# linghaosong/Sextans

Measured on AMD Instinct MI355X. Metric: SpMM GFLOP/s + achieved HBM GB/s (fp32, N=16) at 1/2/4/8 MI355X, higher is better.
Workload: dtype f32; 1 GPU; config4: synthetic CSR 4000000x4000000, Poisson(40) nnz/row, U(-1,1) fp32, N=16, alpha=0.85, beta=-2.06, column-major B/C, seed 4; M=4000000, K=4000000, N=16, nnz=159999547, parallelism=1 GPU

## Files before the change

### sextans_amd/csrc/engine_launch.h

```cpp
#pragma once
#include "engine_state.h"

namespace sxe {

constexpr int kBlock = 256;
constexpr int kWideMaxDict = 576;

void preload_device_code();

void launch_repack(int width, const float *dB, int64_t ldb, float *dBp, int K, int col_base, int ntiles, hipStream_t s, int k_begin = 0,
                   int k_end = -1, int ncols = -1, const unsigned char *touched = nullptr);
void launch_repack_perm(sextans_engine *h, const float *dB, int64_t ldb, float *dBp, int col_base, int ntiles, int ncols, hipStream_t s);
void launch_tiles_to_colmajor(const float *tiles, float *C, int64_t ldc, int M, int col0, int ntiles, int ncols, hipStream_t s);

inline Operands on_panels(const sextans_engine *h, Operands o) {
    o.B = h->d_Bp; o.ldb = h->K; o.layout = BLayout::kPanels;
    return o;
}

void launch_rowgroup(sextans_engine *h, int width, const Operands &o, int ntiles, int row_end, const unsigned char *skip,
                     const int *groups = nullptr, int ngroups = 0);
int launch_panel(sextans_engine *h, int width, const Operands &o, int ntiles, int blk_begin, int blk_end);
enum class V2Order {
    kNatural,
    kBricks,
    kReordered,
    kPositions
};
struct PanelV2 {
    int H = 1;
    V2Order order = V2Order::kNatural;
    int blk_begin = 0, blk_end = -1;
    int last_cols = 16;
    bool dict_blocks_only = false;
};
int launch_panel_v2(sextans_engine *h, const Operands &o, int nsuper, const PanelV2 &a = {});
void launch_window(sextans_engine *h, const Operands &o, int ntiles, int wave_begin, int wave_end);
void launch_colwise(sextans_engine *h, const Operands &o, int N, int row_end);
void launch_chains(sextans_engine *h, const std::vector<Seg> &plan, const Operands &o, int c0, int c1, bool permuted_panels = false);
void launch_hub_pieces(sextans_engine *h, int width, const sextans_engine::PieceTable &t, const Operands &o, int ntiles, int col0, int v0,
                       int v1, const int *colpos = nullptr);
void launch_fold(sextans_engine *h, const sextans_engine::PieceTable &t, int hub0, int hub1, int N, const Operands &o);
void launch_transpose(bool aligned, bool to_cm, const float *src, float *dst, int64_t ld_rm, int64_t ld_cm, int rows, int cols, hipStream_t s);

void launch_rowgroup_bf16(sextans_engine *h, int width, const OperandsBf16 &o, int ntiles);
void launch_hub_pieces_bf16(sextans_engine *h, int width, const sextans_engine::PieceTable &t, const OperandsBf16 &o, int ntiles, int col0, int v0, int v1);
void launch_fold_bf16(sextans_engine *h, const sextans_engine::PieceTable &t, int N, const OperandsBf16 &o);
void launch_widen(const uint16_t *src, int64_t lds, float *dst, int64_t ldd, int64_t rows, int cols, hipStream_t s);
void launch_round(const float *src, int64_t lds, uint16_t *dst, int64_t ldd, int64_t rows, int cols, hipStream_t s);

void launch_chan_unpack_b(const float *ch, int64_t chan_len, int64_t colsize, int num_ch_b, int K, int N, float *B, hipStream_t s);
void launch_chan_unpack_c(const float *ch, int64_t chan_len, int64_t colsize, int M, int N, float *C, hipStream_t s);
void launch_chan_pack_c(const float *C, int M, int N, int64_t chan_len, int64_t colsize, float pad, float *ch, hipStream_t s);

void launch_slab_rows(bool scatter, float *tiles, int64_t tile_stride, const int *rows, int sub, int n, float *slab, int64_t slab_stride, int ntiles, hipStream_t s);

std::vector<Seg> widest_first(int N, int widest);
inline std::vector<Seg> wide_first(int N) { return widest_first(N, 32); }
inline std::vector<Seg> bf16_tiles(int N) { return widest_first(N, 64); }
enum class MainKernel { kRowgroup, kPanel, kWindow, kPanelV2 };
const char *kernel_name(MainKernel main, bool hubs, bool dense);
const char *with_rowblocks(sextans_engine *h, const char *name);

}
```

### sextans_amd/csrc/engine_launch.hip

```cpp
#include <algorithm>

#include "chan_kernels.h"
#include "dispatch.h"
#include "engine_launch.h"
#include "reorder_kernels.h"
#include "spmm_bf16_kernels.h"
#include "spmm_colwise_kernel.h"
#include "spmm_csr_kernels.h"
#include "spmm_panel_v2.h"
#include "spmm_window_kernel.h"

static_assert(sxe::kBlock == sx::kBlock && sxe::kWideMaxDict == sx::kWideMaxDict, "engine_launch.h repeats two constants of the kernel headers");

namespace {
__global__ __launch_bounds__(256) void transpose_tiles(const float *__restrict__ src, int64_t ld_src, float *__restrict__ dst, int64_t ld_dst, int rows, int cols) {
    __shared__ float t[32][33];
    const int c0 = blockIdx.x * 32, r0 = blockIdx.y * 32, tx = threadIdx.x & 31, ty = threadIdx.x >> 5;
    for (int i = ty; i < 32; i += 8)
        if (r0 + i < rows && c0 + tx < cols) t[i][tx] = src[(int64_t)(r0 + i) * ld_src + c0 + tx];
    __syncthreads();
    for (int i = ty; i < 32; i += 8)
        if (c0 + i < cols && r0 + tx < rows) dst[(int64_t)(c0 + i) * ld_dst + r0 + tx] = t[tx][i];
}
template <bool TO_CM, int CW>
// ... 30 lines not shown
        });
    }
}
}

namespace sxe {

void preload_device_code() {
    hipFuncAttributes fa;
    (void)hipFuncGetAttributes(&fa, reinterpret_cast<const void *>(&sx::repack_b_panels<16>));
    (void)hipGetLastError();
}

void launch_repack(int width, const float *dB, int64_t ldb, float *dBp, int K, int col_base, int ntiles, hipStream_t s, int k_begin,
                   int k_end, int ncols, const unsigned char *touched) {
    if (k_end < 0) k_end = K;
    if (k_end <= k_begin) return;
    if (ncols < 0) ncols = ntiles * width;
    dim3 grid((unsigned)((k_end - k_begin + sx::kBlock - 1) / sx::kBlock), (unsigned)ntiles);
    by_width(width, [&](auto L) {
        hipLaunchKernelGGL(sx::repack_b_panels<4 * decltype(L)::value>, grid, dim3(sx::kBlock), 0, s, dB, ldb, dBp, K, col_base, k_begin, k_end, ncols, touched);
    });
}

void launch_repack_perm(sextans_engine *h, const float *dB, int64_t ldb, float *dBp, int col_base, int ntiles, int ncols, hipStream_t s) {
    hipLaunchKernelGGL(sx::repack_b_panels_perm, dim3((unsigned)((h->col_hi - h->col_lo + sx::kBlock - 1) / sx::kBlock), (unsigned)ntiles), dim3(sx::kBlock), 0, s,
                       dB, ldb, dBp, h->K, col_base, h->cluster.d_colpos, h->col_lo, h->col_hi, ncols, h->mat.d_touched);
}

void launch_tiles_to_colmajor(const float *tiles, float *C, int64_t ldc, int M, int col0, int ntiles, int ncols, hipStream_t s) {
    hipLaunchKernelGGL(sx::tiles_to_colmajor, dim3((unsigned)((M + sx::kBlock - 1) / sx::kBlock), (unsigned)ntiles), dim3(sx::kBlock), 0, s, tiles, C, ldc, M, col0, ncols);
}

static int64_t b_stride(const sextans_engine *h, const Operands &o, int NT) { return o.layout == BLayout::kPanels ? (int64_t)h->K * NT : o.ldb; }

void launch_rowgroup(sextans_engine *h, int width, const Operands &o, int ntiles, int row_end, const unsigned char *skip, const int *groups, int ngroups) {
    by_width(width, [&](auto L) {
        constexpr int LPR = decltype(L)::value, RB = sx::kBlock / LPR, CH = 2048;
        const int nrowblk = groups ? ngroups * std::max(1, 128 / RB) : (row_end - o.row_base + RB - 1) / RB;
        if (nrowblk <= 0) return;
        const unsigned nwg = (unsigned)nrowblk * (unsigned)ntiles;
        with_bool(h->opt_exact, [&](auto EX) { with_bool(h->opt_stage, [&](auto ST) { with_bool(o.layout == BLayout::kRowMajor, [&](auto RM) {
            hipLaunchKernelGGL((sx::spmm_csr_rowgroup<LPR, CH, decltype(EX)::value, decltype(ST)::value, decltype(RM)::value>), dim3(nwg), dim3(sx::kBlock), 0,
                               o.s, h->m_rp, h->m_rp + 1, h->m_ci, h->m_v, o.B, b_stride(h, o, 4 * LPR), o.C_in, o.ldc_in, o.C_out, o.ldc, o.row_base, row_end, ntiles, nrowblk,
                               o.alpha, o.beta, (int)h->opt_xcd, skip, groups);
        }); }); });
    });
}

int launch_panel(sextans_engine *h, int width, const Operands &o, int ntiles, int blk_begin, int blk_end) {
    const int nblk = blk_end - blk_begin;
    if (nblk <= 0) return SEXTANS_OK;
    if (int rc = restore_plan_streams(h)) return rc;
    by_width(width, [&](auto L) {
        constexpr int LPR = decltype(L)::value, RB = sx::kBlock / LPR, NT = 4 * LPR;
        const unsigned nwg = (unsigned)nblk * (unsigned)ntiles;
        const int xcd = (int)h->opt_xcd;
        const int pad_rows = h->ps.d_ioff ? sx::kWidePadRows : 1;
        const int panel_floats = (h->ps.plan_pad_row + pad_rows) * NT;
        const int tile_floats = NT * (RB + 1);
        const size_t lds = (size_t)(panel_floats > tile_floats ? panel_floats : tile_floats) * sizeof(int);
        auto go = [&](auto kern) {
            hipLaunchKernelGGL(kern, dim3(nwg), dim3(sx::kBlock), lds, o.s, (const int2 *)h->ps.d_row_off.get(), h->ps.d_lidx,
                               h->ps.d_pcol32, h->ps.d_pval, h->ps.d_blk_row, h->ps.d_dict_ptr, h->ps.d_dict, h->ps.plan_dict_stride, o.B,
                               b_stride(h, o, NT), o.C_in, o.ldc_in, o.C_out, o.ldc, ntiles, nblk, o.alpha, o.beta, xcd, panel_floats,
                               (long long *)h->d_dbg.get(), blk_begin, o.row_base, (const unsigned char *)h->split.d_skip.get(), (const int2 *)h->ps.d_ioff.get(), pad_rows);
        };
        with_bool(h->opt_exact, [&](auto EX) {
            constexpr bool E = decltype(EX)::value;
            if (h->ps.plan_mixed) go(sx::spmm_csr_panel<LPR, E, true>);
            else if (o.layout == BLayout::kColMajor) go(sx::spmm_csr_panel<LPR, E, false, true>);
            else go(sx::spmm_csr_panel<LPR, E, false>);
        });
    });
    return SEXTANS_OK;
}

namespace {
constexpr bool kReorderedContiguous = true;

struct V2Variant {
    int H, NB; bool BCOL, TIMED = false; int DCAP = 9; bool CROW = false, BIG = false; int SETS = 1, RM = 0;
    bool operator==(const V2Variant &o) const {
        return H == o.H && NB == o.NB && BCOL == o.BCOL && TIMED == o.TIMED && DCAP == o.DCAP && CROW == o.CROW && BIG == o.BIG && SETS == o.SETS && RM == o.RM;
    }
};
struct V2Launch {
    int nb, tpw, ngrp, xcd;
    size_t lds;
    int64_t pstride;
    const int *dict, *slot_row;
    const unsigned char *skip;
    V2Variant v;
};

const sextans_engine::PanelState &v2_plan(const sextans_engine *h, V2Order order) { return order == V2Order::kNatural ? h->ps : h->cluster.psc; }

V2Launch plan_panel_v2(const sextans_engine *h, const Operands &o, int nsuper, int nblk, const PanelV2 &a) {
    V2Launch d{};
    const int H = a.H;
    const bool bcol = o.layout == BLayout::kColMajor, rm = o.layout == BLayout::kRowMajor;
    const sextans_engine::PanelState &P = v2_plan(h, a.order);
    d.slot_row = (a.order == V2Order::kBricks || a.order == V2Order::kReordered) ? h->cluster.d_slot_row : nullptr;
    d.skip = a.order == V2Order::kPositions ? nullptr : (const unsigned char *)h->split.d_skip.get();
    const bool crow = a.order == V2Order::kReordered || a.order == V2Order::kPositions;
    const int64_t mean_len = h->M > 0 ? h->m_nnz / h->M : 0;
    int nb = mean_len + 8 <= 32 ? 2 : mean_len + 8 <= 64 ? 4 : 6;
    {
        const int nb_max = std::max(1, (P.plan_max_row + 15) / 16);
        if (nb_max <= nb) nb = nb_max <= 2 ? 2 : nb_max <= 3 ? 3 : nb_max <= 4 ? 4 : 6;
        else if (nb == 2 && nb_max == 3) nb = 3;
    }
    d.nb = nb;
    const bool big = H == 1 && bcol && nb > 2;
    int tpw = (int)h->opt_tiles_per_wg;
    if (tpw <= 0 && big) {
        tpw = std::min<int>(nsuper, std::max<int>(1, (int)(((int64_t)nblk * nsuper + 2 * h->num_cus - 1) / ((int64_t)2 * h->num_cus))));
    } else if (tpw <= 0 && rm && P.plan_sets == 2 && nsuper >= 4) {
        tpw = 1;
    } else if (tpw <= 0) {
        const int64_t rounds = (int64_t)nblk * nsuper / ((int64_t)8 * h->num_cus);
        tpw = (int)std::max<int64_t>(1, std::min<int64_t>(nsuper, rounds));
    }
    d.tpw = std::min(tpw, nsuper);
    d.ngrp = (nsuper + d.tpw - 1) / d.tpw;
    d.pstride = b_stride(h, o, 16);
    d.dict = (rm && crow && h->cluster.d_dict_nat) ? h->cluster.d_dict_nat : P.d_dict;
    const bool small_panel = H == 1 && !bcol && P.plan_pad_row == 5 * 64;
    d.lds = small_panel ? (size_t)(5 * 64 + sx::kWidePadRows) * 64 : (size_t)H * sx::kWideHalfBytes;
    d.xcd = crow && h->opt_reordered_xcd >= 0 ? (int)h->opt_reordered_xcd : (crow && nsuper <= 2 && !kReorderedContiguous) ? 0 : (int)h->opt_xcd;
    V2Variant &v = d.v;
    if (H > 1) { v = {H, 6, bcol}; return d; }
    v = {1, nb, bcol};
    const bool small_dict = bcol && P.plan_max_dict <= 5 * 64 && h->opt_small_v2 != 0;
    if (h->opt_phase_timing && h->d_dbg && h->opt_exact && P.plan_sets == 1) {
        v.TIMED = true;
        if (small_dict && nb == 3) { v.DCAP = 5; return d; }
        if (bcol) { v.NB = 2; return d; }
        if (nb == 6 && !crow && !small_panel) return d;
        if (nb == 2 && !crow && small_panel) { v.DCAP = 5; return d; }
        v.TIMED = false;
    }
    if (small_dict) { v.NB = nb == 3 ? 3 : 2; v.DCAP = 5; }
    else if (big) { v.NB = nb <= 4 ? 4 : 6; v.BIG = true; }
    else if (bcol) v.NB = 2;
    else {
        if (rm) { v.CROW = true; v.RM = (int64_t)h->M * std::max(o.ldc, o.ldc_in) * 4 >= ((int64_t)1 << 32) ? 2 : 1; }
        else v.CROW = crow;
        if (P.plan_sets == 2) { v.NB = 2; v.SETS = 2; }
        else if (small_panel) { v.NB = nb >= 3 ? 3 : 2; v.DCAP = 5; }
    }
    return d;
}

template <int H, int NB, bool BCOL, bool TIMED = false, int DCAP = 9, bool CROW = false, bool BIG = false, int SETS = 1, int RM = 0>
struct V2K {
    static constexpr V2Variant v{H, NB, BCOL, TIMED, DCAP, CROW, BIG, SETS, RM};
    template <class Go>
    static int launch(bool exact, Go &go) {
        if constexpr (TIMED) return go(sx::spmm_csr_panel_v2<H, NB, true, BCOL, TIMED, DCAP, CROW, BIG, SETS, RM>);
        else return with_bool(exact, [&](auto EX) { return go(sx::spmm_csr_panel_v2<H, NB, decltype(EX)::value, BCOL, TIMED, DCAP, CROW, BIG, SETS, RM>); });
    }
};
template <class... Ks>
struct V2List {
    template <class Go>
    static int launch(const V2Variant &v, bool exact, Go &go) {
        int rc = SEXTANS_ERR_STATE;
        const bool found = ((Ks::v == v ? (rc = Ks::launch(exact, go), true) : false) || ...);
        if (!found) g_last_error = "spmm_csr_panel_v2: no instantiation for the variant decided";
        return rc;
    }
};
template <int NB, int DCAP, int SETS, int RM>
using V2Rm = V2K<1, NB, false, false, DCAP, true, false, SETS, RM>;
using PanelV2Kernels = V2List<
    V2K<2, 6, true>, V2K<2, 6, false>,
    V2K<1, 3, true, true, 5>, V2K<1, 2, true, true>, V2K<1, 6, false, true>, V2K<1, 2, false, true, 5>,
    V2K<1, 3, true, false, 5>, V2K<1, 2, true, false, 5>,
    V2K<1, 4, true, false, 9, false, true>, V2K<1, 6, true, false, 9, false, true>,
    V2K<1, 2, true>,
    V2Rm<2, 9, 2, 1>, V2Rm<3, 5, 1, 1>, V2Rm<2, 5, 1, 1>, V2Rm<2, 9, 1, 1>, V2Rm<3, 9, 1, 1>, V2Rm<4, 9, 1, 1>, V2Rm<6, 9, 1, 1>,
    V2Rm<2, 9, 2, 2>, V2Rm<3, 5, 1, 2>, V2Rm<2, 5, 1, 2>, V2Rm<2, 9, 1, 2>, V2Rm<3, 9, 1, 2>, V2Rm<4, 9, 1, 2>, V2Rm<6, 9, 1, 2>,
    V2K<1, 2, false, false, 9, true, false, 2>, V2K<1, 2, false, false, 9, false, false, 2>,
    V2K<1, 3, false, false, 5, true>, V2K<1, 2, false, false, 5, true>,
    V2K<1, 3, false, false, 5>, V2K<1, 2, false, false, 5>,
    V2K<1, 2, false, false, 9, true>, V2K<1, 3, false, false, 9, true>, V2K<1, 4, false, false, 9, true>, V2K<1, 6, false, false, 9, true>,
    V2K<1, 2, false>, V2K<1, 3, false>, V2K<1, 4, false>, V2K<1, 6, false>>;
}

int launch_panel_v2(sextans_engine *h, const Operands &o, int nsuper, const PanelV2 &a) {
    const sextans_engine::PanelState &P = v2_plan(h, a.order);
    const int blk_end = a.blk_end < 0 ? P.plan_nblk : a.blk_end;
    const int nblk = a.dict_blocks_only ? P.n_dict_blocks : blk_end - a.blk_begin;
    if (nblk <= 0 || nsuper <= 0) return SEXTANS_OK;
    if (a.order == V2Order::kNatural)
        if (int rc = restore_plan_streams(h)) return rc;
    const V2Launch d = plan_panel_v2(h, o, nsuper, nblk, a);
    auto go = [&](auto kern) -> int {
        if (int rc = allow_big_lds(h, reinterpret_cast<const void *>(kern), (int)d.lds)) return rc;
        hipLaunchKernelGGL(kern, dim3((unsigned)nblk * (unsigned)d.ngrp), dim3(sx::kBlock), d.lds, o.s, (const int2 *)P.d_row_off.get(),
                           P.d_lidx, P.d_pval, P.d_blk_row, P.d_dict_ptr, d.dict, P.plan_dict_stride, o.B, d.pstride, o.C_in, o.ldc_in, o.C_out, o.ldc, nsuper, d.tpw, nblk, o.alpha, o.beta, d.xcd,
                           P.plan_pad_row, a.blk_begin, o.row_base, d.skip, (long long *)h->d_dbg.get(), d.slot_row, (const int2 *)P.d_ioff.get(), a.last_cols, a.dict_blocks_only ? (const int *)P.d_dict_blocks.get() : (const int *)nullptr);
        return SEXTANS_OK;
    };
    return PanelV2Kernels::launch(d.v, h->opt_exact != 0, go);
}

namespace {
template <bool SCATTER>
__global__ __launch_bounds__(256) void slab_rows(float *tiles, int64_t tile_stride, const int *__restrict__ rows, int sub, int n, float *slab, int64_t slab_stride) {
    const int64_t idx = (int64_t)blockIdx.x * 256 + threadIdx.x;
    const int i = (int)(idx >> 2), q = (int)(idx & 3), t = blockIdx.y;
    if (i >= n) return;
    sx::f32x4 *a = reinterpret_cast<sx::f32x4 *>(tiles + (int64_t)t * tile_stride + (int64_t)(rows[i] - sub) * 16 + 4 * q);
    sx::f32x4 *b = reinterpret_cast<sx::f32x4 *>(slab + (int64_t)t * slab_stride + (int64_t)i * 16 + 4 * q);
    if (SCATTER) *a = *b; else *b = *a;
}
}
void launch_slab_rows(bool scatter, float *tiles, int64_t tile_stride, const int *rows, int sub, int n, float *slab, int64_t slab_stride, int ntiles, hipStream_t s) {
// ... 196 lines not shown
```

### sextans_amd/csrc/engine_spmm.hip

```cpp
#include <algorithm>

#include "engine_launch.h"

using namespace sxe;

namespace sxe {
int fork_chains(sextans_engine *h, const Operands &o, const std::vector<Seg> &segs, int ch0, int ch1) {
    SX_HIP(hipEventRecord(h->ev_fork, o.s));
    SX_HIP(hipStreamWaitEvent(h->aux_stream, h->ev_fork, 0));
    Operands aux = o;
    aux.s = h->aux_stream;
    launch_chains(h, segs, aux, ch0, ch1);
    SX_HIP(hipEventRecord(h->ev_join, h->aux_stream));
    return SEXTANS_OK;
}
}

namespace {
struct RouteCM {
    enum Path { kWindow, kColwise, kSegments } path = kSegments;
    enum Launch { kReorderedV2, kV2Wide, kSplitMixed, kV2, kPanel, kRowgroup };
    bool panel = false;
    int blk0 = 0, blk1 = 0;
    const sextans_engine::PieceTable *pt = nullptr;
// ... 118 lines not shown
        if (r.chains) launch_chains(h, p8, o, r.ch0, r.ch1);
        h->last_kernel = kernel_name(MainKernel::kWindow, r.hubs || r.chains, h->dense.W > 0);
        if (h->dense.rb_n > 0) {
            std::vector<Seg> each;
            for (int t = 0; t < N / 8; ++t) each.push_back(Seg{8, 8 * t, 1});
            if (int rc = launch_rowblocks(h, each, o, N, c.row_end)) return rc;
            h->last_kernel = with_rowblocks(h, h->last_kernel);
        }
    }
    SX_HIP(hipGetLastError());
    return SEXTANS_OK;
}

int run_colwise(sextans_engine *h, const Call &c) {
    Prof p(h, &h->ev_kernel, c.o.s);
    launch_colwise(h, c.o, c.N, c.row_end);
    h->last_kernel = "spmm_csr_colwise";
    SX_HIP(hipGetLastError());
    return SEXTANS_OK;
}

int launch_segment(sextans_engine *h, const Call &c, const RouteCM &r, const Seg &g, RouteCM::Launch l) {
    const Operands panels = on_panels(h, c.o).at(g.col0);
    const Operands src = r.fuse_b ? c.o.at(g.col0) : panels;
    const int *colpos = nullptr;
    PanelV2 a;
    a.blk_begin = r.blk0; a.blk_end = r.blk1;
    switch (l) {
        case RouteCM::kReorderedV2: {
            Operands staged = panels;
            staged.C_in = staged.C_out = h->d_Cs; staged.ldc_in = staged.ldc = r.cs_tile; staged.row_base = 0;
            a = PanelV2{};
            a.order = V2Order::kReordered;
            if (int rc = launch_panel_v2(h, staged, g.ntiles, a))
                return rc;
            colpos = h->cluster.d_colpos;
            break;
        }
        case RouteCM::kV2Wide: {
            const int nsuper = g.ntiles / 2;
            a.H = 2;
            if (int rc = launch_panel_v2(h, src, nsuper, a)) return rc;
            if (g.ntiles & 1)
                if (int rc = launch_panel(h, 16, src.at(nsuper * 32), 1, r.blk0, r.blk1)) return rc;
            break;
        }
        case RouteCM::kSplitMixed:
            a.dict_blocks_only = true;
            if (int rc = launch_panel_v2(h, src, g.ntiles, a)) return rc;
            launch_rowgroup(h, 16, panels, g.ntiles, c.row_end, h->ps.d_rg_skip, h->ps.d_rg_groups, h->ps.rg_ngroups);
            break;
        case RouteCM::kV2:
            if (r.clustered) { a = PanelV2{}; a.order = V2Order::kBricks; }
            if (g.last_cols) a.last_cols = g.last_cols;
            if (int rc = launch_panel_v2(h, src, g.ntiles, a)) return rc;
            break;
        case RouteCM::kPanel:
            if (int rc = launch_panel(h, g.width, src, g.ntiles, r.blk0, r.blk1)) return rc;
            break;
        case RouteCM::kRowgroup:
            launch_rowgroup(h, g.width, panels, g.ntiles, c.row_end, h->split.d_skip);
    }
    if (r.hubs) launch_hub_pieces(h, g.width, *r.pt, panels, g.ntiles, g.col0, r.v0, r.v1, colpos);
    return SEXTANS_OK;
}

int run_segments(sextans_engine *h, const Call &c, const RouteCM &r) {
    const int N = c.N;
    hipStream_t s = c.o.s;
    const Operands panels = on_panels(h, c.o);
    if (!r.skip_repack || r.reordered) {
        Prof p(h, &h->ev_repack, s);
        if (!r.skip_repack) {
            h->bp_layout = r.layout;
            for (const Seg &g : r.segs) {
                float *dst = h->d_Bp + (size_t)h->K * (size_t)g.col0;
                if (r.reordered && g.width == 16 && h->cluster.d_colpos) launch_repack_perm(h, c.o.B, c.o.ldb, dst, g.col0, g.ntiles, g.cols(), s);
                else launch_repack(g.width, c.o.B, c.o.ldb, dst, h->K, g.col0, g.ntiles, s, h->col_lo, h->col_hi, g.cols(), h->mat.d_touched);
            }
        }
        if (r.reordered)
            for (const Seg &g : r.segs)
                if (g.width == 16)
                    launch_repack(16, c.o.C_in, c.o.ldc_in, h->d_Cs, h->M, g.col0, g.ntiles, s, 0, -1, g.cols());
    }
    {
        Prof p(h, &h->ev_kernel, s);
        if (r.chains && !r.reordered)
            if (int rc = fork_chains(h, panels, r.segs, r.ch0, r.ch1)) return rc;
        for (size_t i = 0; i < r.segs.size(); ++i)
            if (int rc = launch_segment(h, c, r, r.segs[i], r.launch[i])) return rc;
        if (r.hubs && !r.reordered) launch_fold(h, *r.pt, r.hub0, r.hub1, N, panels);
        if (r.chains && !r.reordered) SX_HIP(hipStreamWaitEvent(s, h->ev_join, 0));
        const bool v2_used = std::any_of(r.launch, r.launch + r.segs.size(), [](RouteCM::Launch l) { return l < RouteCM::kPanel; });
        h->last_kernel = r.reordered ? "spmm_csr_panel_v2_reordered"
                                     : kernel_name(v2_used ? MainKernel::kPanelV2 : r.panel ? MainKernel::kPanel : MainKernel::kRowgroup, r.hubs || r.chains, h->dense.W > 0);
        if (h->dense.rb_n > 0) {
            if (int rc = launch_rowblocks(h, r.segs, panels, N, c.row_end)) return rc;
            h->last_kernel = with_rowblocks(h, h->last_kernel);
        }
    }
    if (r.reordered) {
        Prof p(h, &h->ev_post, s);
        for (const Seg &g : r.segs)
            if (g.width == 16)
                launch_tiles_to_colmajor(h->d_Cs, c.o.C_out, c.o.ldc, h->M, g.col0, g.ntiles, g.cols(), s);
        if (r.hubs) launch_fold(h, *r.pt, r.hub0, r.hub1, N, panels);
        if (r.chains) launch_chains(h, r.segs, panels, r.ch0, r.ch1, true);
    }
    SX_HIP(hipGetLastError());
    return SEXTANS_OK;
}
}

extern "C" {

int sextans_spmm_device(sextans_handle_t h, int N, float alpha, const float *d_B, int64_t ldb, float beta, const float *d_C_in, float *d_C_out, int64_t ldc, void *stream) {
    return sextans_spmm_device2(h, N, alpha, d_B, ldb, beta, d_C_in, ldc, d_C_out, ldc, stream);
}

int sextans_align_row(sextans_handle_t h, int N, int row, int *aligned) {
    if (!h || !aligned || N <= 0 || (N % 8) != 0 || row < 0 || row > h->M) return SEXTANS_ERR_INVALID;
    if (!h->d_rp) return SEXTANS_ERR_STATE;
    SX_HIP(hipSetDevice(h->device));
    Tiling t;
    if (int rc = prepare(h, N, false, &t)) return rc;
    *aligned = row;
    if (row == h->M) return SEXTANS_OK;
    if (t.window) *aligned = row / h->win.rw * h->win.rw;
    else if (t.panel && !h->ps.h_blk_row.empty())
        *aligned = *(std::upper_bound(h->ps.h_blk_row.begin(), h->ps.h_blk_row.end(), row) - 1);
    return SEXTANS_OK;
}

int sextans_spmm_device2(sextans_handle_t h, int N, float alpha, const float *d_B, int64_t ldb,
                         float beta, const float *d_C_in, int64_t ldc_in, float *d_C_out, int64_t ldc, void *stream) {
    if (!h) return SEXTANS_ERR_INVALID;
    return sextans_spmm_device_rows(h, N, alpha, d_B, ldb, beta, d_C_in, ldc_in, d_C_out, ldc, 0, h->M, 0, stream);
}
// ... 38 lines not shown
```

### sextans_amd/csrc/reorder_kernels.h

```cpp
#pragma once
#include <hip/hip_runtime.h>
#include <stdint.h>

#include "spmm_csr_kernels.h"

namespace sx {

__global__ __launch_bounds__(kBlock) void repack_b_panels_perm(const float *__restrict__ B, int64_t ldb, float *__restrict__ Bp, int K,
                                                               int col_base, const int *__restrict__ colpos, int k_begin, int k_end, int ncols,
                                                               const unsigned char *__restrict__ touched) {
    __shared__ float s[16][kBlock + 1];
    const int tid = threadIdx.x;
    const int k0 = k_begin + blockIdx.x * kBlock;
    const int t = blockIdx.y;
    const float *src = B + (int64_t)(col_base + t * 16) * ldb;
    if (touched && !(touched[k0 >> 6] | touched[(k0 >> 6) + 1] | touched[(k0 >> 6) + 2] | touched[(k0 >> 6) + 3])) return;
    if ((t + 1) * 16 > ncols) {
        if (k0 + tid < k_end)
            for (int c = 0; c < 16; ++c) s[c][tid] = t * 16 + c < ncols ? src[(int64_t)c * ldb + k0 + tid] : 0.f;
    } else if (k0 + tid < k_end) {
#pragma unroll
        for (int c = 0; c < 16; ++c) s[c][tid] = src[(int64_t)c * ldb + k0 + tid];
    }
    __syncthreads();
// ... 15 lines not shown
    __shared__ __attribute__((aligned(16))) float s[16 * LD];
    const int tid = threadIdx.x;
    const int r0 = blockIdx.x * kBlock;
    const int t = blockIdx.y;
    const float *src = Cs + (int64_t)t * M * 16 + (int64_t)r0 * 16;
    const int nr = min(kBlock, M - r0);
#pragma unroll
    for (int i = 0; i < 4; ++i) {
        const int e4 = tid + i * kBlock;
        const int rr = e4 >> 2, c4 = (e4 & 3) * 4;
        if (rr < nr) {
            const f32x4 v = *reinterpret_cast<const f32x4 *>(src + (int64_t)e4 * 4);
            s[(c4 + 0) * LD + rr] = v.x; s[(c4 + 1) * LD + rr] = v.y; s[(c4 + 2) * LD + rr] = v.z; s[(c4 + 3) * LD + rr] = v.w;
        }
    }
    __syncthreads();
    float *dst = C + (int64_t)(col_base + t * 16) * ldc + r0;
#pragma unroll
    for (int i = 0; i < 4; ++i) {
        const int g = tid + i * kBlock;
        const int c = g >> 6, rr = (g & 63) * 4;
        if (t * 16 + c >= ncols) continue;
        float *d = dst + (int64_t)c * ldc + rr;
        if (rr + 3 < nr) {
            const f32x4 v = *reinterpret_cast<const f32x4 *>(&s[c * LD + rr]);
            if ((reinterpret_cast<uintptr_t>(d) & 15) == 0) *reinterpret_cast<f32x4 *>(d) = v;
            else { d[0] = v.x; d[1] = v.y; d[2] = v.z; d[3] = v.w; }
        } else {
            for (int k = 0; rr + k < nr; ++k) d[k] = s[c * LD + rr + k];
        }
    }
}

}
```

### sextans_amd/csrc/spmm_panel_v2.h

```cpp
#pragma once
#include <hip/hip_runtime.h>
#include <stdint.h>

#include "spmm_csr_kernels.h"

namespace sx {

constexpr int kWideMaxDict = 576;
constexpr int kWidePadRows = 16;
constexpr int kWideHalfBytes = (kWideMaxDict + kWidePadRows) * 64;

template <int G>
__device__ __forceinline__ int quad_bcast(int x) {
    return __builtin_amdgcn_update_dpp(0, x, G * 0x55, 0xF, 0xF, true);
}

template <bool EXACT>
__device__ __forceinline__ void mac4v(f32x4 &acc, float a, const f32x4 &b) {
    acc.x = mac<EXACT>(acc.x, a, b.x);
    acc.y = mac<EXACT>(acc.y, a, b.y);
    acc.z = mac<EXACT>(acc.z, a, b.z);
    acc.w = mac<EXACT>(acc.w, a, b.w);
}

// ... 23 lines not shown

template <int H, bool EXACT>
__device__ __forceinline__ void wide_batch(const int (&ix)[4], const float (&vx)[4], const char *pq, f32x4 (&acc)[H]) {
    wide_quad<0, H, EXACT>(ix, vx, pq, acc); pin<H>(acc);
    wide_quad<1, H, EXACT>(ix, vx, pq, acc); pin<H>(acc);
    wide_quad<2, H, EXACT>(ix, vx, pq, acc); pin<H>(acc);
    wide_quad<3, H, EXACT>(ix, vx, pq, acc); pin<H>(acc);
}

__device__ __forceinline__ void glds16(const float *gsrc, char *lds_dst) {
    __builtin_amdgcn_global_load_lds((const __attribute__((address_space(1))) void *)gsrc,
                                     (__attribute__((address_space(3))) void *)lds_dst, 16, 0, 0);
}

__device__ __forceinline__ void aload4(f32x4 &dst, const float *sbase, unsigned voff_bytes) {
    asm volatile("global_load_dwordx4 %0, %1, %2" : "=v"(dst) : "v"(voff_bytes), "s"(sbase) : "memory");
}
__device__ __forceinline__ void aload1(float &dst, const float *sbase, unsigned voff_bytes) {
    asm volatile("global_load_dword %0, %1, %2" : "=v"(dst) : "v"(voff_bytes), "s"(sbase) : "memory");
}
__device__ __forceinline__ void astore1(float *sbase, unsigned voff_bytes, float val) {
    asm volatile("global_store_dword %0, %1, %2" : : "v"(voff_bytes), "v"(val), "s"(sbase) : "memory");
}
__device__ __forceinline__ void astore4(float *sbase, unsigned voff_bytes, const f32x4 &val) {
    asm volatile("global_store_dwordx4 %0, %1, %2" : : "v"(voff_bytes), "v"(val), "s"(sbase) : "memory");
}
__device__ __forceinline__ void aload4p(f32x4 &dst, const float *p) {
    asm volatile("global_load_dwordx4 %0, %1, off" : "=v"(dst) : "v"(p) : "memory");
}
__device__ __forceinline__ void astore4p(float *p, const f32x4 &val) {
    asm volatile("global_store_dwordx4 %0, %1, off" : : "v"(p), "v"(val) : "memory");
}

template <int H, int NB, bool EXACT, bool BCOL, bool TIMED = false, int DCAP = 9, bool CROW = false, bool BIG = false, int SETS = 1, int RM = 0>
#ifndef SX_V2_BCOL_WGS
#define SX_V2_BCOL_WGS 3
#endif
__global__ __launch_bounds__(kBlock, (H == 1 && !BIG ? (BCOL && DCAP == 9 ? SX_V2_BCOL_WGS : 4) : 2)) void spmm_csr_panel_v2(
    const int2 *__restrict__ slot_info, const unsigned short *__restrict__ p_idx16, const float *__restrict__ p_val,
    const int *__restrict__ blk_row, const int *__restrict__ dict_cnt, const int *__restrict__ blk_dict, int dict_stride,
    const float *__restrict__ Bp, int64_t panel_stride, const float *Cin, int64_t ldc_in, float *Cout, int64_t ldc,
    int nsuper, int tpw, int nblk, float alpha, float beta, int use_xcd_remap, int pad_row, int blk_begin, int row_base,
    const unsigned char *__restrict__ skip, long long *dbg, const int *__restrict__ slot_row, const int2 *__restrict__ slot_ioff, int last_cols,
    const int *__restrict__ blk_list) {
    static_assert(!CROW || (H == 1 && !BCOL), "the block-major C staging exists for 16-column tiles on repacked panels");
    static_assert(!RM || (CROW && !TIMED && !BIG), "row-major operands use the 16-byte C accesses of the staging form");
    static_assert(SETS == 1 || (H == 1 && !BCOL && !TIMED && !BIG && NB <= 2), "several row sets per block: 16-column tiles on repacked panels, short rows");
    long long t0 = 0, t1 = 0, t2 = 0, t3 = 0, w0 = 0;
    if constexpr (TIMED) { t0 = clock64(); w0 = wall_clock64(); }
    constexpr int LPR = 4;
    constexpr int RB = kBlock / LPR;
    constexpr int RBS = RB * SETS;
    constexpr int NTT = 16 * H;
    constexpr int BATCH = 16;
    constexpr int MAXD = DCAP;
    extern __shared__ __attribute__((aligned(16))) int smem[];
    char *lds = reinterpret_cast<char *>(smem);

    const int ngrp = (nsuper + tpw - 1) / tpw;
    const unsigned nwg = (unsigned)nblk * (unsigned)ngrp;
    unsigned wg = blockIdx.x;
    if (use_xcd_remap) wg = xcd_remap(wg, nwg);
    const int blk = blk_list ? blk_list[wg / (unsigned)ngrp] : blk_begin + (int)(wg / (unsigned)ngrp);
    const int grp = (int)(wg % (unsigned)ngrp);
    const int st_begin = grp * tpw, st_end = min(nsuper, st_begin + tpw);

    const int tid = threadIdx.x;
    const int slot = tid / LPR;
    const int q = tid % LPR;
    const int row0 = blk_row[blk];
    const int row1 = blk_row[blk + 1];
    const int nu = dict_cnt[blk];
    int2 si[SETS], io2[SETS];
#pragma unroll
    for (int t = 0; t < SETS; ++t) {
        si[t] = slot_info[(int64_t)blk * RBS + t * RB + slot];
        io2[t] = slot_ioff ? slot_ioff[(int64_t)blk * RBS + t * RB + slot] : make_int2(si[t].x, 0);
    }
    unsigned boff[MAXD];
// ... 119 lines not shown
        cvoff_rin[t] = RM ? (coff[t] * (unsigned)ldc_in + 4u * (unsigned)q) * 4u : ((unsigned)myrow[t] * 16u + 4u * (unsigned)q) * 4u;
        cvoff_rout[t] = RM ? (coff[t] * (unsigned)ldc + 4u * (unsigned)q) * 4u : cvoff_rin[t];
    }
    const int64_t ct_in = RM ? 16 : ldc_in, ct_out = RM ? 16 : ldc;
    constexpr bool kRematC = RM == 1 && SETS == 2;
    auto off_rin = [&](int t) -> unsigned {
        if constexpr (kRematC) { unsigned c = coff[t]; asm volatile("" : "+v"(c)); return (c * (unsigned)ldc_in + 4u * (unsigned)q) * 4u; }
        else return cvoff_rin[t];
    };
    auto off_rout = [&](int t) -> unsigned {
        if constexpr (kRematC) { unsigned c = coff[t]; asm volatile("" : "+v"(c)); return (c * (unsigned)ldc + 4u * (unsigned)q) * 4u; }
        else return cvoff_rout[t];
    };
    const float *cp_in[SETS];
    float *cp_out[SETS];
#pragma unroll
    for (int t = 0; t < SETS; ++t) {
        cp_in[t] = Cin + (int64_t)coff[t] * ldc_in + 4 * q;
        cp_out[t] = Cout + (int64_t)coff[t] * ldc + 4 * q;
    }
    auto ptr_in = [&](int t) -> const float * {
        if constexpr (RM == 2 && SETS == 2) { unsigned c = coff[t]; asm volatile("" : "+v"(c)); return Cin + (int64_t)c * ldc_in + 4 * q; }
        else return cp_in[t];
    };
    auto ptr_out = [&](int t) -> float * {
        if constexpr (RM == 2 && SETS == 2) { unsigned c = coff[t]; asm volatile("" : "+v"(c)); return Cout + (int64_t)c * ldc + 4 * q; }
        else return cp_out[t];
    };
    float cin[SETS][H][4];
    f32x4 cinv[SETS];
#pragma unroll
    for (int t = 0; t < SETS; ++t) {
        cinv[t] = f32x4{0.f, 0.f, 0.f, 0.f};
        if constexpr (CROW) {
            if (!RM || cvalid || st_begin + 1 < nsuper) {
                if constexpr (RM == 2) aload4p(cinv[t], ptr_in(t) + (int64_t)st_begin * 16);
                else aload4(cinv[t], Cin + (int64_t)st_begin * ct_in, off_rin(t));
            }
        } else if (cvalid || st_begin + 1 < nsuper) {
#pragma unroll
            for (int h = 0; h < H; ++h)
#pragma unroll
                for (int j = 0; j < 4; ++j) aload1(cin[t][h][j], Cin + ((int64_t)st_begin * NTT + h * 16 + j) * ldc_in, cvoff_in[t]);
        }
    }
    if constexpr (!DMA) store_panel();
#pragma unroll
    for (int t = 0; t < SETS; ++t)
#pragma unroll
        for (int b = 0; b < NB; ++b) asm volatile("" : "+v"(av[t][b]));
    __syncthreads();
    asm volatile("s_waitcnt vmcnt(0)" ::: "memory");
    if constexpr (TIMED) t2 = clock64();
    long long t_rows = 0;
    for (int st = st_begin; st < st_end; ++st) {
        const int64_t col0 = (int64_t)st * NTT;
        if constexpr (DMA) {
            if (st != st_begin) {
                __syncthreads();
                dma_panel(st);
                __syncthreads();
            }
        }
        if (st != st_begin) {
#pragma unroll
            for (int t = 0; t < SETS; ++t) {
                if constexpr (CROW) {
                    if (!RM || cvalid || st + 1 < nsuper) {
                        if constexpr (RM == 2) aload4p(cinv[t], ptr_in(t) + (int64_t)st * 16);
                        else aload4(cinv[t], Cin + (int64_t)st * ct_in, off_rin(t));
                    }
                } else if (cvalid || st + 1 < nsuper) {
#pragma unroll
                    for (int h = 0; h < H; ++h)
#pragma unroll
                        for (int j = 0; j < 4; ++j) aload1(cin[t][h][j], Cin + (col0 + h * 16 + j) * ldc_in, cvoff_in[t]);
                }
            }
        }
        if constexpr (!DMA) {
            if (st + 1 < st_end) load_panel(st + 1, false);
        }
        f32x4 acc[SETS][H];
#pragma unroll
        for (int t = 0; t < SETS; ++t) {
#pragma unroll
        for (int h = 0; h < H; ++h) acc[t][h] = f32x4{0.f, 0.f, 0.f, 0.f};
#define SX_RBATCH(b)                                                                                  \
        if constexpr ((b) < NB) {                                                                      \
        if (__builtin_amdgcn_ballot_w64(len[t] >= ((b) + 1) * BATCH) == __builtin_amdgcn_ballot_w64(true)) { \
            float vb[4] = {av[t][b].x, av[t][b].y, av[t][b].z, av[t][b].w};                            \
            wide_batch<H, EXACT>(ai[t][b], vb, pq[t], acc[t]);                                         \
        } else if (len[t] > (b) * BATCH) {                                                            \
            float vb[4] = {av[t][b].x, av[t][b].y, av[t][b].z, av[t][b].w};                            \
            const int cnt = len[t] - (b) * BATCH;                                                      \
            wide_quad<0, H, EXACT>(ai[t][b], vb, pq[t], acc[t]); pin<H>(acc[t]);                       \
            if (cnt > 4) { wide_quad<1, H, EXACT>(ai[t][b], vb, pq[t], acc[t]); pin<H>(acc[t]); }      \
            if (cnt > 8) { wide_quad<2, H, EXACT>(ai[t][b], vb, pq[t], acc[t]); pin<H>(acc[t]); }      \
            if (cnt > 12) { wide_quad<3, H, EXACT>(ai[t][b], vb, pq[t], acc[t]); pin<H>(acc[t]); }     \
        }                                                                                              \
        }
        SX_RBATCH(0) SX_RBATCH(1) SX_RBATCH(2) SX_RBATCH(3) SX_RBATCH(4) SX_RBATCH(5)
#undef SX_RBATCH
        for (int pos = NB * BATCH; pos < len[t]; pos += BATCH) {
            const f32x4 v = *reinterpret_cast<const f32x4 *>(pv + loff[t] + pos);
            const uint2 w = *reinterpret_cast<const uint2 *>(pi + loffi[t] + pos);
            int ix[4] = {(int)(w.x & 0xffffu), (int)(w.x >> 16), (int)(w.y & 0xffffu), (int)(w.y >> 16)};
            float vx[4] = {v.x, v.y, v.z, v.w};
            const int cnt = len[t] - pos;
            wide_quad<0, H, EXACT>(ix, vx, pq[t], acc[t]); pin<H>(acc[t]);
            if (cnt > 4) { wide_quad<1, H, EXACT>(ix, vx, pq[t], acc[t]); pin<H>(acc[t]); }
            if (cnt > 8) { wide_quad<2, H, EXACT>(ix, vx, pq[t], acc[t]); pin<H>(acc[t]); }
            if (cnt > 12) { wide_quad<3, H, EXACT>(ix, vx, pq[t], acc[t]); pin<H>(acc[t]); }
        }
        }

        if constexpr (TIMED) {
            asm volatile("" : "+v"(acc[0][0]) : : "memory");
            t_rows += clock64() - (st == st_begin ? t2 : t3);
        }
        if constexpr (H == 2) {
            asm volatile("s_waitcnt vmcnt(0)"
                         : "+v"(cin[0][0][0]), "+v"(cin[0][0][1]), "+v"(cin[0][0][2]), "+v"(cin[0][0][3]), "+v"(cin[0][1][0]), "+v"(cin[0][1][1]),
                           "+v"(cin[0][1][2]), "+v"(cin[0][1][3])
                         :
                         : "memory");
        } else if constexpr (CROW && SETS == 2) {
            asm volatile("s_waitcnt vmcnt(0)" : "+v"(cinv[0]), "+v"(cinv[SETS - 1]) : : "memory");
        } else if constexpr (CROW) {
            asm volatile("s_waitcnt vmcnt(0)" : "+v"(cinv[0]) : : "memory");
        } else if constexpr (SETS == 2) {
            asm volatile("s_waitcnt vmcnt(0)"
                         : "+v"(cin[0][0][0]), "+v"(cin[0][0][1]), "+v"(cin[0][0][2]), "+v"(cin[0][0][3]), "+v"(cin[SETS - 1][0][0]),
                           "+v"(cin[SETS - 1][0][1]), "+v"(cin[SETS - 1][0][2]), "+v"(cin[SETS - 1][0][3])
                         :
                         : "memory");
        } else {
            static_assert((H == 1 || H == 2) && SETS <= 2, "the drain names the C_in registers explicitly");
            asm volatile("s_waitcnt vmcnt(0)" : "+v"(cin[0][0][0]), "+v"(cin[0][0][1]), "+v"(cin[0][0][2]), "+v"(cin[0][0][3]) : : "memory");
        }
        if constexpr (!DMA) {
#pragma unroll
            for (int u = 0; u < MAXD; ++u)
#pragma unroll
                for (int h = 0; h < H; ++h) {
                    if constexpr (BCOL) asm volatile("" : "+v"(bs[u][h][0]), "+v"(bs[u][h][1]), "+v"(bs[u][h][2]), "+v"(bs[u][h][3]));
                    else asm volatile("" : "+v"(bv[u][h]));
                }
        }
#pragma unroll
        for (int t = 0; t < SETS; ++t) {
            if constexpr (CROW) {
                if (cwrite[t] && (!RM || cvalid || st + 1 < nsuper)) {
                    const f32x4 o = {epilogue<EXACT>(alpha, acc[t][0].x, beta, cinv[t].x), epilogue<EXACT>(alpha, acc[t][0].y, beta, cinv[t].y),
                                     epilogue<EXACT>(alpha, acc[t][0].z, beta, cinv[t].z), epilogue<EXACT>(alpha, acc[t][0].w, beta, cinv[t].w)};
                    if constexpr (RM == 2) astore4p(ptr_out(t) + (int64_t)st * 16, o);
                    else astore4(Cout + (int64_t)st * ct_out, off_rout(t), o);
                }
            } else if (cwrite[t] && (cvalid || st + 1 < nsuper)) {
#pragma unroll
                for (int h = 0; h < H; ++h) {
                    const float a4[4] = {acc[t][h].x, acc[t][h].y, acc[t][h].z, acc[t][h].w};
#pragma unroll
                    for (int j = 0; j < 4; ++j)
                        astore1(Cout + (col0 + h * 16 + j) * ldc, cvoff_out[t], epilogue<EXACT>(alpha, a4[j], beta, cin[t][h][j]));
                }
            }
        }
        if constexpr (!DMA) {
            if (st + 1 < st_end) {
                __syncthreads();
                store_panel();
                __syncthreads();
            }
        }
        if constexpr (TIMED) t3 = clock64();
    }
    if constexpr (TIMED) {
        asm volatile("s_waitcnt vmcnt(0)" ::: "memory");
        const long long t4 = clock64();
        if (dbg && tid == 0 && (blockIdx.x & 15) == 5) {
            atomicAdd((unsigned long long *)&dbg[0], (unsigned long long)(t1 - t0));
            atomicAdd((unsigned long long *)&dbg[1], (unsigned long long)(t2 - t1));
            atomicAdd((unsigned long long *)&dbg[2], (unsigned long long)t_rows);
            atomicAdd((unsigned long long *)&dbg[3], (unsigned long long)(t4 - t2 - t_rows));
            atomicAdd((unsigned long long *)&dbg[4], 1ull);
// ... 7 lines not shown
```

Before: 1633 GFLOP/s.

## Defer alpha/beta epilogue of reordered panel path into the colmajor write-back pass

Measured after the change: 1634 GFLOP/s, median of 4. No clear change (+0.0%).

```diff
diff --git a/sextans_amd/csrc/engine_launch.h b/sextans_amd/csrc/engine_launch.h
--- a/sextans_amd/csrc/engine_launch.h
+++ b/sextans_amd/csrc/engine_launch.h
@@ -12,6 +12,7 @@
                    int k_end = -1, int ncols = -1, const unsigned char *touched = nullptr);
 void launch_repack_perm(sextans_engine *h, const float *dB, int64_t ldb, float *dBp, int col_base, int ntiles, int ncols, hipStream_t s);
 void launch_tiles_to_colmajor(const float *tiles, float *C, int64_t ldc, int M, int col0, int ntiles, int ncols, hipStream_t s);
+void launch_tiles_to_colmajor_epilogue(sextans_engine *h, const float *tiles, const Operands &o, int col0, int ntiles, int ncols);
 
 inline Operands on_panels(const sextans_engine *h, Operands o) {
     o.B = h->d_Bp; o.ldb = h->K; o.layout = BLayout::kPanels;
@@ -33,6 +34,7 @@
     int blk_begin = 0, blk_end = -1;
     int last_cols = 16;
     bool dict_blocks_only = false;
+    bool defer_epilogue = false;
 };
 int launch_panel_v2(sextans_engine *h, const Operands &o, int nsuper, const PanelV2 &a = {});
 void launch_window(sextans_engine *h, const Operands &o, int ntiles, int wave_begin, int wave_end);
diff --git a/sextans_amd/csrc/engine_launch.hip b/sextans_amd/csrc/engine_launch.hip
--- a/sextans_amd/csrc/engine_launch.hip
+++ b/sextans_amd/csrc/engine_launch.hip
@@ -86,6 +86,13 @@
     hipLaunchKernelGGL(sx::tiles_to_colmajor, dim3((unsigned)((M + sx::kBlock - 1) / sx::kBlock), (unsigned)ntiles), dim3(sx::kBlock), 0, s, tiles, C, ldc, M, col0, ncols);
 }
 
+void launch_tiles_to_colmajor_epilogue(sextans_engine *h, const float *tiles, const Operands &o, int col0, int ntiles, int ncols) {
+    with_bool(h->opt_exact, [&](auto EX) {
+        hipLaunchKernelGGL(sx::tiles_to_colmajor_epilogue<decltype(EX)::value>, dim3((unsigned)((h->M + sx::kBlock - 1) / sx::kBlock), (unsigned)ntiles), dim3(sx::kBlock), 0, o.s,
+                           tiles, o.C_in, o.ldc_in, o.C_out, o.ldc, h->M, col0, ncols, o.alpha, o.beta, (const unsigned char *)h->split.d_skip.get());
+    });
+}
+
 static int64_t b_stride(const sextans_engine *h, const Operands &o, int NT) { return o.layout == BLayout::kPanels ? (int64_t)h->K * NT : o.ldb; }
 
 void launch_rowgroup(sextans_engine *h, int width, const Operands &o, int ntiles, int row_end, const unsigned char *skip, const int *groups, int ngroups) {
@@ -134,9 +141,10 @@
 constexpr bool kReorderedContiguous = true;
 
 struct V2Variant {
-    int H, NB; bool BCOL, TIMED = false; int DCAP = 9; bool CROW = false, BIG = false; int SETS = 1, RM = 0;
+    int H, NB; bool BCOL, TIMED = false; int DCAP = 9; bool CROW = false, BIG = false; int SETS = 1, RM = 0; bool DEFER = false;
     bool operator==(const V2Variant &o) const {
-        return H == o.H && NB == o.NB && BCOL == o.BCOL && TIMED == o.TIMED && DCAP == o.DCAP && CROW == o.CROW && BIG == o.BIG && SETS == o.SETS && RM == o.RM;
+        return H == o.H && NB == o.NB && BCOL == o.BCOL && TIMED == o.TIMED && DCAP == o.DCAP && CROW == o.CROW && BIG == o.BIG && SETS == o.SETS && RM == o.RM &&
+               DEFER == o.DEFER;
     }
 };
 struct V2Launch {
@@ -200,20 +208,20 @@
     else if (bcol) v.NB = 2;
     else {
         if (rm) { v.CROW = true; v.RM = (int64_t)h->M * std::max(o.ldc, o.ldc_in) * 4 >= ((int64_t)1 << 32) ? 2 : 1; }
-        else v.CROW = crow;
+        else { v.CROW = crow; v.DEFER = crow && a.defer_epilogue; }
         if (P.plan_sets == 2) { v.NB = 2; v.SETS = 2; }
         else if (small_panel) { v.NB = nb >= 3 ? 3 : 2; v.DCAP = 5; }
     }
     return d;
 }
 
-template <int H, int NB, bool BCOL, bool TIMED = false, int DCAP = 9, bool CROW = false, bool BIG = false, int SETS = 1, int RM = 0>
+template <int H, int NB, bool BCOL, bool TIMED = false, int DCAP = 9, bool CROW = false, bool BIG = false, int SETS = 1, int RM = 0, bool DEFER = false>
 struct V2K {
-    static constexpr V2Variant v{H, NB, BCOL, TIMED, DCAP, CROW, BIG, SETS, RM};
+    static constexpr V2Variant v{H, NB, BCOL, TIMED, DCAP, CROW, BIG, SETS, RM, DEFER};
     template <class Go>
     static int launch(bool exact, Go &go) {
-        if constexpr (TIMED) return go(sx::spmm_csr_panel_v2<H, NB, true, BCOL, TIMED, DCAP, CROW, BIG, SETS, RM>);
-        else return with_bool(exact, [&](auto EX) { return go(sx::spmm_csr_panel_v2<H, NB, decltype(EX)::value, BCOL, TIMED, DCAP, CROW, BIG, SETS, RM>); });
+        if constexpr (TIMED) return go(sx::spmm_csr_panel_v2<H, NB, true, BCOL, TIMED, DCAP, CROW, BIG, SETS, RM, DEFER>);
+        else return with_bool(exact, [&](auto EX) { return go(sx::spmm_csr_panel_v2<H, NB, decltype(EX)::value, BCOL, TIMED, DCAP, CROW, BIG, SETS, RM, DEFER>); });
     }
 };
 template <class... Ks>
@@ -228,6 +236,8 @@
 };
 template <int NB, int DCAP, int SETS, int RM>
 using V2Rm = V2K<1, NB, false, false, DCAP, true, false, SETS, RM>;
+template <int NB, int DCAP = 9, int SETS = 1>
+using V2Defer = V2K<1, NB, false, false, DCAP, true, false, SETS, 0, true>;
 using PanelV2Kernels = V2List<
     V2K<2, 6, true>, V2K<2, 6, false>,
     V2K<1, 3, true, true, 5>, V2K<1, 2, true, true>, V2K<1, 6, false, true>, V2K<1, 2, false, true, 5>,
@@ -240,6 +250,7 @@
     V2K<1, 3, false, false, 5, true>, V2K<1, 2, false, false, 5, true>,
     V2K<1, 3, false, false, 5>, V2K<1, 2, false, false, 5>,
     V2K<1, 2, false, false, 9, true>, V2K<1, 3, false, false, 9, true>, V2K<1, 4, false, false, 9, true>, V2K<1, 6, false, false, 9, true>,
+    V2Defer<2, 9, 2>, V2Defer<3, 5>, V2Defer<2, 5>, V2Defer<2>, V2Defer<3>, V2Defer<4>, V2Defer<6>,
     V2K<1, 2, false>, V2K<1, 3, false>, V2K<1, 4, false>, V2K<1, 6, false>>;
 }
 
diff --git a/sextans_amd/csrc/engine_spmm.hip b/sextans_amd/csrc/engine_spmm.hip
--- a/sextans_amd/csrc/engine_spmm.hip
+++ b/sextans_amd/csrc/engine_spmm.hip
@@ -174,6 +174,7 @@
             staged.C_in = staged.C_out = h->d_Cs; staged.ldc_in = staged.ldc = r.cs_tile; staged.row_base = 0;
             a = PanelV2{};
             a.order = V2Order::kReordered;
+            a.defer_epilogue = true;
             if (int rc = launch_panel_v2(h, staged, g.ntiles, a))
                 return rc;
             colpos = h->cluster.d_colpos;
@@ -211,20 +212,14 @@
     const int N = c.N;
     hipStream_t s = c.o.s;
     const Operands panels = on_panels(h, c.o);
-    if (!r.skip_repack || r.reordered) {
+    if (!r.skip_repack) {
         Prof p(h, &h->ev_repack, s);
-        if (!r.skip_repack) {
-            h->bp_layout = r.layout;
-            for (const Seg &g : r.segs) {
-                float *dst = h->d_Bp + (size_t)h->K * (size_t)g.col0;
-                if (r.reordered && g.width == 16 && h->cluster.d_colpos) launch_repack_perm(h, c.o.B, c.o.ldb, dst, g.col0, g.ntiles, g.cols(), s);
-                else launch_repack(g.width, c.o.B, c.o.ldb, dst, h->K, g.col0, g.ntiles, s, h->col_lo, h->col_hi, g.cols(), h->mat.d_touched);
-            }
-        }
-        if (r.reordered)
-            for (const Seg &g : r.segs)
-                if (g.width == 16)
-                    launch_repack(16, c.o.C_in, c.o.ldc_in, h->d_Cs, h->M, g.col0, g.ntiles, s, 0, -1, g.cols());
+        h->bp_layout = r.layout;
+        for (const Seg &g : r.segs) {
+            float *dst = h->d_Bp + (size_t)h->K * (size_t)g.col0;
+            if (r.reordered && g.width == 16 && h->cluster.d_colpos) launch_repack_perm(h, c.o.B, c.o.ldb, dst, g.col0, g.ntiles, g.cols(), s);
+            else launch_repack(g.width, c.o.B, c.o.ldb, dst, h->K, g.col0, g.ntiles, s, h->col_lo, h->col_hi, g.cols(), h->mat.d_touched);
+        }
     }
     {
         Prof p(h, &h->ev_kernel, s);
@@ -246,7 +241,7 @@
         Prof p(h, &h->ev_post, s);
         for (const Seg &g : r.segs)
             if (g.width == 16)
-                launch_tiles_to_colmajor(h->d_Cs, c.o.C_out, c.o.ldc, h->M, g.col0, g.ntiles, g.cols(), s);
+                launch_tiles_to_colmajor_epilogue(h, h->d_Cs, c.o, g.col0, g.ntiles, g.cols());
         if (r.hubs) launch_fold(h, *r.pt, r.hub0, r.hub1, N, panels);
         if (r.chains) launch_chains(h, r.segs, panels, r.ch0, r.ch1, true);
     }
diff --git a/sextans_amd/csrc/reorder_kernels.h b/sextans_amd/csrc/reorder_kernels.h
--- a/sextans_amd/csrc/reorder_kernels.h
+++ b/sextans_amd/csrc/reorder_kernels.h
@@ -71,4 +71,75 @@
     }
 }
 
+template <bool EXACT>
+__global__ __launch_bounds__(kBlock) void tiles_to_colmajor_epilogue(const float *__restrict__ Cs, const float *Cin, int64_t ldc_in, float *Cout,
+                                                                     int64_t ldc, int M, int col_base, int ncols, float alpha, float beta,
+                                                                     const unsigned char *__restrict__ skip) {
+    constexpr int LD = kBlock + 4;
+    __shared__ __attribute__((aligned(16))) float s[16 * LD];
+    const int tid = threadIdx.x;
+    const int r0 = blockIdx.x * kBlock;
+    const int t = blockIdx.y;
+    const int nr = min(kBlock, M - r0);
+    const float *cbase = Cin + (int64_t)(col_base + t * 16) * ldc_in + r0;
+    f32x4 cin[4];
+    unsigned sk[4];
+#pragma unroll
+    for (int i = 0; i < 4; ++i) {
+        const int g = tid + i * kBlock;
+        const int c = g >> 6, rr = (g & 63) * 4;
+        cin[i] = f32x4{0.f, 0.f, 0.f, 0.f};
+        sk[i] = 0;
+        if (t * 16 + c >= ncols) continue;
+        const float *p = cbase + (int64_t)c * ldc_in + rr;
+        if (rr + 3 < nr) {
+            if ((reinterpret_cast<uintptr_t>(p) & 15) == 0) cin[i] = *reinterpret_cast<const f32x4 *>(p);
+            else cin[i] = f32x4{p[0], p[1], p[2], p[3]};
+            if (skip) sk[i] = *reinterpret_cast<const unsigned *>(skip + r0 + rr);
+        } else {
+            float x[4] = {0.f, 0.f, 0.f, 0.f};
+#pragma unroll
+            for (int k = 0; k < 4; ++k)
+                if (rr + k < nr) {
+                    x[k] = p[k];
+                    if (skip) sk[i] |= (unsigned)skip[r0 + rr + k] << (8 * k);
+                }
+            cin[i] = f32x4{x[0], x[1], x[2], x[3]};
+        }
+    }
+    const float *src = Cs + (int64_t)t * M * 16 + (int64_t)r0 * 16;
+#pragma unroll
+    for (int i = 0; i < 4; ++i) {
+        const int e4 = tid + i * kBlock;
+        const int rr = e4 >> 2, c4 = (e4 & 3) * 4;
+        if (rr < nr) {
+            const f32x4 v = *reinterpret_cast<const f32x4 *>(src + (int64_t)e4 * 4);
+            s[(c4 + 0) * LD + rr] = v.x; s[(c4 + 1) * LD + rr] = v.y; s[(c4 + 2) * LD + rr] = v.z; s[(c4 + 3) * LD + rr] = v.w;
+        }
+    }
+    __syncthreads();
+    float *dst = Cout + (int64_t)(col_base + t * 16) * ldc + r0;
+#pragma unroll
+    for (int i = 0; i < 4; ++i) {
+        const int g = tid + i * kBlock;
+        const int c = g >> 6, rr = (g & 63) * 4;
+        if (t * 16 + c >= ncols) continue;
+        float *d = dst + (int64_t)c * ldc + rr;
+        const f32x4 a = *reinterpret_cast<const f32x4 *>(&s[c * LD + rr]);
+        const f32x4 v = {(sk[i] & 0xffu) ? cin[i].x : epilogue<EXACT>(alpha, a.x, beta, cin[i].x),
+                         (sk[i] & 0xff00u) ? cin[i].y : epilogue<EXACT>(alpha, a.y, beta, cin[i].y),
+                         (sk[i] & 0xff0000u) ? cin[i].z : epilogue<EXACT>(alpha, a.z, beta, cin[i].z),
+                         (sk[i] & 0xff000000u) ? cin[i].w : epilogue<EXACT>(alpha, a.w, beta, cin[i].w)};
+        if (rr + 3 < nr) {
+            if ((reinterpret_cast<uintptr_t>(d) & 15) == 0) *reinterpret_cast<f32x4 *>(d) = v;
+            else { d[0] = v.x; d[1] = v.y; d[2] = v.z; d[3] = v.w; }
+        } else {
+            const float x[4] = {v.x, v.y, v.z, v.w};
+#pragma unroll
+            for (int k = 0; k < 4; ++k)
+                if (rr + k < nr) d[k] = x[k];
+        }
+    }
 }
+
+}
diff --git a/sextans_amd/csrc/spmm_panel_v2.h b/sextans_amd/csrc/spmm_panel_v2.h
--- a/sextans_amd/csrc/spmm_panel_v2.h
+++ b/sextans_amd/csrc/spmm_panel_v2.h
@@ -79,7 +79,8 @@
     asm volatile("global_store_dwordx4 %0, %1, off" : : "v"(p), "v"(val) : "memory");
 }
 
-template <int H, int NB, bool EXACT, bool BCOL, bool TIMED = false, int DCAP = 9, bool CROW = false, bool BIG = false, int SETS = 1, int RM = 0>
+template <int H, int NB, bool EXACT, bool BCOL, bool TIMED = false, int DCAP = 9, bool CROW = false, bool BIG = false, int SETS = 1, int RM = 0,
+          bool DEFER = false>
 #ifndef SX_V2_BCOL_WGS
 #define SX_V2_BCOL_WGS 3
 #endif
@@ -92,6 +93,7 @@
     const int *__restrict__ blk_list) {
     static_assert(!CROW || (H == 1 && !BCOL), "the block-major C staging exists for 16-column tiles on repacked panels");
     static_assert(!RM || (CROW && !TIMED && !BIG), "row-major operands use the 16-byte C accesses of the staging form");
+    static_assert(!DEFER || (CROW && RM == 0), "the deferred epilogue belongs to the write-back pass of the staging buffer");
     static_assert(SETS == 1 || (H == 1 && !BCOL && !TIMED && !BIG && NB <= 2), "several row sets per block: 16-column tiles on repacked panels, short rows");
     long long t0 = 0, t1 = 0, t2 = 0, t3 = 0, w0 = 0;
     if constexpr (TIMED) { t0 = clock64(); w0 = wall_clock64(); }
@@ -277,7 +279,8 @@
 #pragma unroll
     for (int t = 0; t < SETS; ++t) {
         cinv[t] = f32x4{0.f, 0.f, 0.f, 0.f};
-        if constexpr (CROW) {
+        if constexpr (DEFER) {
+        } else if constexpr (CROW) {
             if (!RM || cvalid || st_begin + 1 < nsuper) {
                 if constexpr (RM == 2) aload4p(cinv[t], ptr_in(t) + (int64_t)st_begin * 16);
                 else aload4(cinv[t], Cin + (int64_t)st_begin * ct_in, off_rin(t));
@@ -310,7 +313,8 @@
         if (st != st_begin) {
 #pragma unroll
             for (int t = 0; t < SETS; ++t) {
-                if constexpr (CROW) {
+                if constexpr (DEFER) {
+                } else if constexpr (CROW) {
                     if (!RM || cvalid || st + 1 < nsuper) {
                         if constexpr (RM == 2) aload4p(cinv[t], ptr_in(t) + (int64_t)st * 16);
                         else aload4(cinv[t], Cin + (int64_t)st * ct_in, off_rin(t));
@@ -370,6 +374,8 @@
                            "+v"(cin[0][1][2]), "+v"(cin[0][1][3])
                          :
                          : "memory");
+        } else if constexpr (DEFER) {
+            asm volatile("s_waitcnt vmcnt(0)" ::: "memory");
         } else if constexpr (CROW && SETS == 2) {
             asm volatile("s_waitcnt vmcnt(0)" : "+v"(cinv[0]), "+v"(cinv[SETS - 1]) : : "memory");
         } else if constexpr (CROW) {
@@ -396,7 +402,9 @@
 #pragma unroll
         for (int t = 0; t < SETS; ++t) {
             if constexpr (CROW) {
-                if (cwrite[t] && (!RM || cvalid || st + 1 < nsuper)) {
+                if constexpr (DEFER) {
+                    if (cwrite[t]) astore4(Cout + (int64_t)st * ct_out, off_rout(t), acc[t][0]);
+                } else if (cwrite[t] && (!RM || cvalid || st + 1 < nsuper)) {
                     const f32x4 o = {epilogue<EXACT>(alpha, acc[t][0].x, beta, cinv[t].x), epilogue<EXACT>(alpha, acc[t][0].y, beta, cinv[t].y),
                                      epilogue<EXACT>(alpha, acc[t][0].z, beta, cinv[t].z), epilogue<EXACT>(alpha, acc[t][0].w, beta, cinv[t].w)};
                     if constexpr (RM == 2) astore4p(ptr_out(t) + (int64_t)st * 16, o);
```
